# zhangganlin/GlORIE-SLAM

Measured on AMD Instinct MI355X. Metric: DSPO BA-update iters/sec + rendered rays/sec, 640x480 Replica keyframe graph, higher is better.
Workload: dtype f16 corr/ConvGRU, f32 Jacobians, f64 solve; render: f32 (decoder matmuls as 3-term f16 splits, f32 accumulate); 1 GPU; G8: 8 keyframes, 36 edges, 60x80 (640x480/8), BA itrs=2, DSPO stages alternating, context part of the GRU gates (one map per source keyframe) re-evaluated for all keyframes every 12 steps; multiview_filter.thresh = 0.25 (reference ships 0.01, configs/mono_point_slam.yaml:75: with untrained weights 0.01 rejects > 80 % of every frame and no depth_scale step would reach stage 2); render: 524k-point c; edges_local=36, edges_total=36, hw=4800, keyframes=8, parallelism=single GPU

## Files before the change

### glorie_slam_amd/csrc/conv.hip

```cpp
#include <hip/hip_runtime.h>
#include <stdint.h>
#include <stdlib.h>
#include <string.h>
#include <type_traits>
#include "common.hiph"

namespace glorie {

typedef __attribute__((ext_vector_type(8))) _Float16 f16x8;
typedef __attribute__((ext_vector_type(4))) _Float16 f16x4;
typedef __attribute__((ext_vector_type(4))) float f32x4;

enum { EPI_BIAS_ACT = 0, EPI_GRU_ZR = 1, EPI_GRU_Q = 2, EPI_GLO = 3, EPI_HEADS = 4, EPI_UPSAMPLE = 5 };
enum { CACT_NONE = 0, CACT_RELU = 1, CACT_SIGMOID = 2 };

struct ConvArgs {
  const _Float16* xa; int xa_stride; int cha;
  const _Float16* xb; int xb_stride; int chb;
  const _Float16* w;
  int taps, npad, nout;
  long P; int H, W, HW;
  _Float16* out; int out_stride;
  _Float16* out2; int out2_stride;
  const float* terms; int terms_stride; int act;
  const _Float16* net; int net_stride;
  const _Float16* z; int z_stride;
  const _Float16* pre; int pre_stride;
  const int* pre_map;
  long pbeg;
  int pair;
  unsigned long long* stamps;
  int pp_full, pp_nbr;
  const f16x8* tap_w; float* tap_out; int tap_groups, tap_ncols;
  const float* up_disps; const int64_t* up_ix; float* up_out; int up_f32;
};

constexpr int kTileN = 128;
constexpr long kConvPpwMinPixels = 512L * 512;

__device__ __forceinline__ float csigmoid(float x) { return __builtin_amdgcn_rcpf(1.0f + __expf(-x)); }
__device__ __forceinline__ float ctanh(float x) {
  const float e = __expf(-2.0f * fabsf(x));
  return copysignf((1.0f - e) * __builtin_amdgcn_rcpf(1.0f + e), x);
}

__device__ __forceinline__ void glds16(const void* src, char* lds_wave_base) {
  __builtin_amdgcn_global_load_lds((const __attribute__((address_space(1))) void*)src,
                                   (__attribute__((address_space(3))) void*)lds_wave_base, 16, 0, 0);
}

__device__ __forceinline__ long pre_pixel(const ConvArgs& a, long p) {
  if (!a.pre_map) return p;
  const int e = (int)(p / a.HW);
  return (long)a.pre_map[e] * a.HW + (p - (long)e * a.HW);
}

template <int EPI>
__device__ __forceinline__ void conv_epilogue(const ConvArgs& a, const f32x4 v, long p, int e, int n) {
  f16x4 o;
  if (EPI == EPI_BIAS_ACT) {
    float4 b = make_float4(0.f, 0.f, 0.f, 0.f);
    if (a.terms) b = *reinterpret_cast<const float4*>(a.terms + n);
    float f[4] = {v[0] + b.x, v[1] + b.y, v[2] + b.z, v[3] + b.w};
#pragma unroll
    for (int k = 0; k < 4; ++k) {
      if (a.act == CACT_RELU) f[k] = fmaxf(f[k], 0.0f);
      else if (a.act == CACT_SIGMOID) f[k] = csigmoid(f[k]);
      o[k] = (_Float16)f[k];
    }
    *reinterpret_cast<f16x4*>(a.out + p * a.out_stride + n) = o;
  } else if (EPI == EPI_GRU_ZR) {
    const float4 g = *reinterpret_cast<const float4*>(a.terms + (size_t)e * a.terms_stride + n);
    const float s[4] = {csigmoid(v[0] + g.x), csigmoid(v[1] + g.y), csigmoid(v[2] + g.z),
                        csigmoid(v[3] + g.w)};
    if (n < 128) {
#pragma unroll
      for (int k = 0; k < 4; ++k) o[k] = (_Float16)s[k];
      *reinterpret_cast<f16x4*>(a.out + p * a.out_stride + n) = o;
    } else {
      const f16x4 nv = *reinterpret_cast<const f16x4*>(a.net + p * a.net_stride + (n - 128));
#pragma unroll
      for (int k = 0; k < 4; ++k) o[k] = (_Float16)(s[k] * (float)nv[k]);
      *reinterpret_cast<f16x4*>(a.out2 + p * a.out2_stride + (n - 128)) = o;
    }
  } else {
    const float4 g = *reinterpret_cast<const float4*>(a.terms + (size_t)e * a.terms_stride + n);
    const f16x4 nv = *reinterpret_cast<const f16x4*>(a.net + p * a.net_stride + n);
    const f16x4 zv = *reinterpret_cast<const f16x4*>(a.z + p * a.z_stride + n);
    const float qv[4] = {ctanh(v[0] + g.x), ctanh(v[1] + g.y), ctanh(v[2] + g.z), ctanh(v[3] + g.w)};
#pragma unroll
    for (int k = 0; k < 4; ++k) {
      const float zz = (float)zv[k];
      o[k] = (_Float16)((1.0f - zz) * (float)nv[k] + zz * qv[k]);
    }
    *reinterpret_cast<f16x4*>(a.out + p * a.out_stride + n) = o;
  }
}

typedef __attribute__((ext_vector_type(2))) unsigned u32x2;

typedef __attribute__((ext_vector_type(4))) unsigned u32x4e;

template <int EPI, int MB, int NB>
__device__ __forceinline__ void conv_epilogue_pair(const ConvArgs& a, f32x4 (&acc)[MB][NB], long pbase, int nwave) {
  static_assert(MB % 2 == 0, "pairs of 16-row blocks");
  constexpr int PB = MB / 2;
  const int kg = (threadIdx.x & 63) >> 4;
  const __amdgpu_buffer_rsrc_t rO = __builtin_amdgcn_make_buffer_rsrc((void*)a.out, 0, 0x7fffffff, 0x00020000);
  const __amdgpu_buffer_rsrc_t rO2 = __builtin_amdgcn_make_buffer_rsrc((void*)(EPI == EPI_GRU_ZR ? a.out2 : a.out), 0,
                                                                      0x7fffffff, 0x00020000);
  const bool upper = EPI == EPI_GRU_ZR && nwave >= 128;
  const bool late = EPI != EPI_BIAS_ACT && a.pre;
  int nch[PB];
#pragma unroll
  for (int b = 0; b < PB; ++b) nch[b] = min(nwave + 32 * b + 8 * kg, a.nout - 8);
  float4 g[PB][2];
  int e_cur = -1;
  if (EPI == EPI_BIAS_ACT) {
#pragma unroll
    for (int b = 0; b < PB; ++b) {
      g[b][0] = a.terms ? *reinterpret_cast<const float4*>(a.terms + nch[b]) : make_float4(0.f, 0.f, 0.f, 0.f);
      g[b][1] = a.terms ? *reinterpret_cast<const float4*>(a.terms + nch[b] + 4) : make_float4(0.f, 0.f, 0.f, 0.f);
    }
// ... 183 lines not shown
    for (int rb = 0; rb < 2; ++rb) {
      f32x4 s = f32x4{0.f, 0.f, 0.f, 0.f};
#pragma unroll
      for (int c = 0; c < 2; ++c) s = __builtin_amdgcn_mfma_f32_16x16x32_f16(wf[c][rb], hf[c], s, 0, 0, 0);
      t[rb][ni] = s;
    }
  }
  float* red = reinterpret_cast<float*>(smem);
  __syncthreads();
  if (wm == 1) {
#pragma unroll
    for (int rb = 0; rb < 2; ++rb)
#pragma unroll
      for (int ni = 0; ni < NB; ++ni)
#pragma unroll
        for (int r = 0; r < 4; ++r) red[((wn * 8 + rb * 4 + ni) * 4 + r) * 64 + lane] = t[rb][ni][r];
  }
  __syncthreads();
  if (wm == 0) {
#pragma unroll
    for (int ni = 0; ni < NB; ++ni) {
      const long p = p0 + wn * 64 + ni * 16 + col;
      if (p >= a.P) continue;
      float* dst = a.tap_out + (size_t)(grp * a.tap_ncols) * a.P + p;
#pragma unroll
      for (int rb = 0; rb < 2; ++rb) {
        const int n = rb * 16 + kg * 4;
#pragma unroll
        for (int r = 0; r < 4; ++r) {
          const float v = t[rb][ni][r] + red[((wn * 8 + rb * 4 + ni) * 4 + r) * 64 + lane];
          if (n + r < a.tap_ncols) dst[(size_t)(n + r) * a.P] = v;
        }
      }
    }
  }
}

template <int MB, int NB>
__device__ __forceinline__ void conv_epilogue_glo(const ConvArgs& a, f32x4 (&acc)[MB][NB], long p0, long pbase, int wm,
                                                  int wn, int kg, int col, char* smem, int tile) {
  static_assert(MB == 4, "128-channel tile");
  const long pend = (p0 / a.HW + 1) * a.HW;
  float s0[MB][4];
#pragma unroll
  for (int mi = 0; mi < MB; ++mi)
#pragma unroll
    for (int k = 0; k < 4; ++k) s0[mi][k] = 0.0f;
  const int nb = wm * 64 + kg * 4;
#pragma unroll
  for (int ni = 0; ni < NB; ++ni) {
    const long p = pbase + ni * 16;
    const bool okp = p < pend;
    const long pc = okp ? p : pend - 1;
#pragma unroll
    for (int mi = 0; mi < MB; ++mi) {
      const int n = nb + mi * 16;
      const float4 b = *reinterpret_cast<const float4*>(a.terms + n);
      const f16x4 nv = *reinterpret_cast<const f16x4*>(a.net + pc * a.net_stride + n);
      const f32x4 v = acc[mi][ni];
      s0[mi][0] += okp ? csigmoid(v[0] + b.x) * (float)nv[0] : 0.0f;
      s0[mi][1] += okp ? csigmoid(v[1] + b.y) * (float)nv[1] : 0.0f;
      s0[mi][2] += okp ? csigmoid(v[2] + b.z) * (float)nv[2] : 0.0f;
      s0[mi][3] += okp ? csigmoid(v[3] + b.w) * (float)nv[3] : 0.0f;
    }
  }
#pragma unroll
  for (int mi = 0; mi < MB; ++mi)
#pragma unroll
    for (int k = 0; k < 4; ++k)
#pragma unroll
      for (int off = 8; off > 0; off >>= 1) s0[mi][k] += __shfl_xor(s0[mi][k], off, 64);
  float* red = reinterpret_cast<float*>(smem);
  __syncthreads();
  if (col == 0) {
#pragma unroll
    for (int mi = 0; mi < MB; ++mi)
#pragma unroll
      for (int k = 0; k < 4; ++k) red[wn * 128 + nb + mi * 16 + k] = s0[mi][k];
  }
  __syncthreads();
  const int tid = threadIdx.x;
  if (tid < 128) reinterpret_cast<float*>(a.out)[(size_t)tile * 128 + tid] = red[tid] + red[128 + tid];
}

__device__ __forceinline__ float round_prob(float v, bool f32) { return f32 ? v : (float)(_Float16)v; }

template <int MB, int NB>
__device__ __forceinline__ void conv_epilogue_upsample(const ConvArgs& a, f32x4 (&acc)[MB][NB], long p0, int n0, int wm,
                                                       int wn, int kg, int col, char* smem) {
  static_assert(MB == 4 && NB == 4, "128 x 128 tile");
  _Float16* T = reinterpret_cast<_Float16*>(smem);
  float4 bias[MB];
#pragma unroll
  for (int mi = 0; mi < MB; ++mi) bias[mi] = *reinterpret_cast<const float4*>(a.terms + n0 + wm * 64 + mi * 16 + kg * 4);
  __syncthreads();
#pragma unroll
  for (int ni = 0; ni < NB; ++ni) {
    const int pl = wn * 64 + ni * 16 + col;
#pragma unroll
    for (int mi = 0; mi < MB; ++mi) {
      const int b = wm * 4 + mi;
      const f32x4 v = acc[mi][ni];
      const f16x4 h = {(_Float16)(v[0] + bias[mi].x), (_Float16)(v[1] + bias[mi].y), (_Float16)(v[2] + bias[mi].z),
                       (_Float16)(v[3] + bias[mi].w)};
      *reinterpret_cast<f16x4*>(T + pl * 128 + ((b ^ (pl & 7)) * 16 + kg * 4)) = h;
    }
  }
  __syncthreads();
  const int tid = threadIdx.x;
  const int pl = tid & 127, hb = tid >> 7;
  const long p = p0 + pl;
  if (p >= a.P) return;
  const int asub = n0 >> 7;
  const int m = (int)(p / a.HW);
  const int q = (int)(p - (long)m * a.HW);
  const int y = q / a.W, x = q - y * a.W;
  const int frame = (int)a.up_ix[m];
  const float* dmap = a.up_disps + (size_t)frame * a.HW;
  float nb[9];
#pragma unroll
  for (int k = 0; k < 9; ++k) {
    const int yy = y + k / 3 - 1, xx = x + k % 3 - 1;
    const bool in = yy >= 0 && yy < a.H && xx >= 0 && xx < a.W;
    nb[k] = dmap[in ? yy * a.W + xx : q];
    if (!in) nb[k] = 0.0f;
  }
  float outv[4];
#pragma unroll
  for (int j = 0; j < 4; ++j) {
    const int b = hb * 4 + j;
    const f16x8* src = reinterpret_cast<const f16x8*>(T + pl * 128 + (b ^ (pl & 7)) * 16);
    const f16x8 lo = src[0], hi = src[1];
    float v[9];
#pragma unroll
    for (int k = 0; k < 8; ++k) v[k] = (float)lo[k];
    v[8] = (float)hi[0];
    float mx = v[0];
#pragma unroll
    for (int k = 1; k < 9; ++k) mx = fmaxf(mx, v[k]);
    float e[9], sum = 0.0f;
#pragma unroll
    for (int k = 0; k < 9; ++k) { e[k] = expf(v[k] - mx); sum += e[k]; }
    float o = 0.0f;
#pragma unroll
    for (int k = 0; k < 9; ++k)
      o = __fadd_rn(o, __fmul_rn(round_prob(e[k] / sum, a.up_f32 != 0), nb[k]));
    outv[j] = o;
  }
  float* dst = a.up_out + (size_t)frame * 64 * a.HW + (size_t)(8 * y + asub) * (8 * a.W) + 8 * x + hb * 4;
  *reinterpret_cast<float4*>(dst) = make_float4(outv[0], outv[1], outv[2], outv[3]);
}

template <int EPI, int NB, int BK, int NW, int ST, int MB = 4>
__global__ __launch_bounds__(64 * NW, (ST == 1 && MB * NB <= 16) ? 3 : 2) void conv_igemm_kernel(ConvArgs a) {
  constexpr int TN = 32 * MB;
  static_assert(ST == 1 || ST == 2, "LDS stages");
#if defined(__HIP_DEVICE_COMPILE__)
  constexpr int PT = (NW / 2) * 16 * NB;
  constexpr int RB = BK * 2;
  constexpr int SL = RB / 16;
  constexpr int RPI = 64 / SL;
  constexpr int XI = PT / RPI / NW;
  constexpr int WI = TN / RPI / NW;
  constexpr int XBYTES = PT * RB, WBYTES = TN * RB;
  constexpr int KK = BK / 32;
  extern __shared__ __attribute__((aligned(16))) char smem[];
  const int tid = threadIdx.x, lane = tid & 63, wv = tid >> 6;
  const int col = lane & 15, kg = lane >> 4;
// ... 911 lines not shown
  long rest_px = a.P - full_pt * 512;
  int nbr = 4;
  long rest_pt = 0;
  if (rest_px > 0) {
    const long per_cu = (rest_px * ntn + ncu - 1) / ncu;
    nbr = (int)((per_cu + 127) / 128);
    if (nbr > 4 || full_pt == 0) nbr = 4;
    if (nbr < 1) nbr = 1;
    rest_pt = (rest_px + 128 * nbr - 1) / (128 * nbr);
  }
  if (nbr == 4) { full_pt = pt_all; rest_pt = 0; }
  const long nwg = (full_pt + rest_pt) * ntn;
  if (nwg <= 0) return GLORIE_OK;
  if (nwg > 0x7fffffffL) return GLORIE_EINVAL;
  a.pp_full = (int)(full_pt * ntn);
  a.pp_nbr = nbr;
  const dim3 grid((unsigned)nwg);
  switch (epilogue) {
    case EPI_BIAS_ACT: launch_ppw_one<EPI_BIAS_ACT>(a, grid, st); break;
    case EPI_GRU_Q: launch_ppw_one<EPI_GRU_Q>(a, grid, st); break;
    case EPI_HEADS: launch_ppw_one<EPI_HEADS>(a, grid, st); break;
    default: return GLORIE_EUNSUPPORTED;
  }
  return check_launch();
}

template <int MB>
static int launch_conv_halo(const ConvArgs& a, int epilogue, hipStream_t st) {
  constexpr int PT = 128, TN = 32 * MB;
  if (a.pair && (MB % 2)) return GLORIE_EINVAL;
  const long ptiles = (a.P - a.pbeg + PT - 1) / PT;
  if (ptiles <= 0) return GLORIE_OK;
  const long nwg = ptiles * ((a.nout + TN - 1) / TN);
  if (nwg > 0x7fffffffL) return GLORIE_EINVAL;
  const dim3 grid((unsigned)nwg);
  const size_t lds = halo_lds_bytes(a.W, MB);
  switch (epilogue) {
    case EPI_BIAS_ACT: launch_halo_one<EPI_BIAS_ACT, MB>(a, grid, lds, st); break;
    case EPI_GRU_ZR: launch_halo_one<EPI_GRU_ZR, MB>(a, grid, lds, st); break;
    case EPI_GRU_Q:
      if constexpr (MB == 4) launch_halo_one<EPI_GRU_Q, MB>(a, grid, lds, st);
      else return GLORIE_EUNSUPPORTED;
      break;
    case EPI_HEADS:
      if constexpr (MB == 4) launch_halo_one<EPI_HEADS, MB>(a, grid, lds, st);
      else return GLORIE_EUNSUPPORTED;
      break;
    default: return GLORIE_EUNSUPPORTED;
  }
  return check_launch();
}

template <int NB, int BK, int NW, int ST, int MB = 4>
static int launch_conv(const ConvArgs& a, int epilogue, hipStream_t st, long max_ptiles = -1) {
  constexpr int PT = (NW / 2) * 16 * NB;
  if (a.pair && (MB % 2)) return GLORIE_EINVAL;
  long ptiles = (a.P - a.pbeg + PT - 1) / PT;
  if (epilogue == EPI_GLO) ptiles = (a.P / a.HW) * ((a.HW + PT - 1) / PT);
  if (max_ptiles >= 0) ptiles = ptiles < max_ptiles ? ptiles : max_ptiles;
  if (ptiles <= 0) return GLORIE_OK;
  const long nwg = ptiles * ((a.nout + 32 * MB - 1) / (32 * MB));
  if (nwg > 0x7fffffffL) return GLORIE_EINVAL;
  const dim3 grid((unsigned)nwg);
  switch (epilogue) {
    case EPI_BIAS_ACT: launch_one<EPI_BIAS_ACT, NB, BK, NW, ST, MB>(a, grid, st); break;
    case EPI_GRU_ZR: launch_one<EPI_GRU_ZR, NB, BK, NW, ST, MB>(a, grid, st); break;
    case EPI_GLO:
      if constexpr (MB == 4 && NB == 4 && NW == 4 && ST == 1) launch_one<EPI_GLO, NB, BK, NW, ST, MB>(a, grid, st);
      else return GLORIE_EUNSUPPORTED;
      break;
    case EPI_HEADS:
      if constexpr (MB == 4 && NB == 4 && NW == 4 && ST == 1) launch_one<EPI_HEADS, NB, BK, NW, ST, MB>(a, grid, st);
      else return GLORIE_EUNSUPPORTED;
      break;
    case EPI_UPSAMPLE:
      if constexpr (MB == 4 && NB == 4 && NW == 4 && ST == 1) launch_one<EPI_UPSAMPLE, NB, BK, NW, ST, MB>(a, grid, st);
      else return GLORIE_EUNSUPPORTED;
      break;
    default: launch_one<EPI_GRU_Q, NB, BK, NW, ST, MB>(a, grid, st); break;
  }
  return check_launch();
}

}

using namespace glorie;

static int conv_igemm_impl(const void* xa, int xa_stride, int ca, const void* xb, int xb_stride,
                           int cb, const void* w_packed, int taps, int nout, int epilogue,
                           const float* terms, int terms_stride, int act, const void* net,
                           int net_stride, const void* z, int z_stride, void* out, int out_stride,
                           void* out2, int out2_stride, const void* pre, int pre_stride, const int* pre_map,
                           int N, int H, int W, void* stream, const void* tap_w, float* tap_out, int tap_groups,
                           int tap_ncols, const float* up_disps = nullptr, const int64_t* up_ix = nullptr,
                           float* up_out = nullptr, int up_f32 = 0) {
  if (N < 0 || H <= 0 || W <= 0 || (taps != 1 && taps != 9) || nout <= 0 || (nout & 3)) return GLORIE_EINVAL;
  if (ca < 0 || cb < 0 || (ca % 64) || (cb % 64) || ca + cb == 0) return GLORIE_EINVAL;
  const int pair = (epilogue >> 8) & 1;
  const int policy = (epilogue >> 12) & 15;
  epilogue &= 0xff;
  if (policy > 7) return GLORIE_EINVAL;
  if (epilogue < 0 || epilogue > 5) return GLORIE_EINVAL;
  if (pair && (epilogue > EPI_GRU_Q || (nout & 31))) return GLORIE_EINVAL;
  if (epilogue == EPI_UPSAMPLE && (!up_disps || !up_ix || !up_out || !terms || nout != 1024 || taps != 1 || pre))
    return GLORIE_EINVAL;
  if (epilogue == EPI_HEADS && (!tap_w || !tap_out || !terms || tap_groups < 1 || tap_ncols < 1 || tap_ncols > 32 ||
                                nout < 128 * tap_groups || (nout & 127) || act != CACT_RELU || pre))
    return GLORIE_EINVAL;
  if (N == 0) return GLORIE_OK;
  if ((ca && (!xa || (xa_stride & 7))) || (cb && (!xb || (xb_stride & 7)))) return GLORIE_EINVAL;
  if (!w_packed || !out || (out_stride & 3)) return GLORIE_EINVAL;
  if (epilogue == EPI_GRU_ZR && (nout != 256 || !terms || !net || !out2 || (terms_stride & 3))) return GLORIE_EINVAL;
  if (epilogue == EPI_GRU_Q && (nout != 128 || !terms || !net || !z || (terms_stride & 3))) return GLORIE_EINVAL;
  if (pre && (epilogue == EPI_BIAS_ACT || epilogue == EPI_GLO || (pre_stride & 3))) return GLORIE_EINVAL;
  if (epilogue == EPI_GLO && (nout != 128 || taps != 1 || !terms || !net)) return GLORIE_EINVAL;
  ConvArgs a;
  a.xa = reinterpret_cast<const _Float16*>(xa); a.xa_stride = xa_stride; a.cha = ca / 64;
  a.xb = reinterpret_cast<const _Float16*>(xb); a.xb_stride = xb_stride; a.chb = cb / 64;
  a.w = reinterpret_cast<const _Float16*>(w_packed);
  a.taps = taps; a.nout = nout; a.npad = (nout + kTileN - 1) / kTileN * kTileN;
  a.P = (long)N * H * W; a.H = H; a.W = W; a.HW = H * W;
  a.out = reinterpret_cast<_Float16*>(out); a.out_stride = out_stride;
  a.out2 = reinterpret_cast<_Float16*>(out2); a.out2_stride = out2_stride;
  a.terms = terms; a.terms_stride = terms_stride; a.act = act;
  a.net = reinterpret_cast<const _Float16*>(net); a.net_stride = net_stride;
  a.z = reinterpret_cast<const _Float16*>(z); a.z_stride = z_stride;
  a.pre = reinterpret_cast<const _Float16*>(pre); a.pre_stride = pre_stride; a.pre_map = pre ? pre_map : nullptr;
  a.pbeg = 0;
  a.tap_w = reinterpret_cast<const f16x8*>(tap_w); a.tap_out = tap_out; a.tap_groups = tap_groups;
  a.tap_ncols = tap_ncols;
  a.up_disps = up_disps; a.up_ix = up_ix; a.up_out = up_out; a.up_f32 = up_f32;
  a.pair = pair;
  a.pp_full = 0; a.pp_nbr = 4;
#ifdef EXP_CONV_STAMPS
  a.stamps = getenv("GLORIE_CONV_STAMPS") ? (unsigned long long*)strtoull(getenv("GLORIE_CONV_STAMPS"), nullptr, 0) : nullptr;
#else
  a.stamps = nullptr;
#endif
  const long lim = 0x7fffffffL;
  if (((a.P + W + 2) * (long)xa_stride + 64) * 2 > lim || ((a.P + W + 2) * (long)xb_stride + 64) * 2 > lim ||
      ((long)taps * a.npad * (ca + cb) + 64) * 2 > lim || (pre && (a.P * (long)pre_stride + 512) * 2 > lim) ||
      (a.P * (long)out_stride + nout) * 2 > lim || (out2 && (a.P * (long)out2_stride + 128) * 2 > lim))
    return GLORIE_EINVAL;
  hipStream_t st = (hipStream_t)stream;
  if (policy == 6) return launch_conv_pp(a, epilogue, st);
  if (policy == 7) return launch_conv_ppw(a, epilogue, st);
  {
    const char* ppw = getenv("GLORIE_CONV_PPW");
    const bool fits = (nout & 127) == 0 && (epilogue == EPI_BIAS_ACT || epilogue == EPI_GRU_Q || epilogue == EPI_HEADS);
    const bool want = ppw ? ppw[0] == '1' : (taps == 9 && (nout == 128 || epilogue == EPI_HEADS) && epilogue != EPI_BIAS_ACT &&
                                             a.P >= kConvPpwMinPixels);
    if (policy == 0 && fits && want && !(ppw && ppw[0] == '0')) return launch_conv_ppw(a, epilogue, st);
  }
  {
    if (policy == 0 && taps == 9 && a.pbeg == 0) {
      const long tiles128 = (a.P + 127) / 128 * ((nout + 127) / 128);
      if (nout > 64 && (nout & 255) != 0 && W <= 83 && (epilogue <= EPI_GRU_Q || epilogue == EPI_HEADS) &&
          !(epilogue == EPI_BIAS_ACT && tiles128 <= 384))
        return launch_conv_halo<4>(a, epilogue, st);
    }
  }
  if (epilogue == EPI_HEADS || epilogue == EPI_UPSAMPLE) return launch_conv<4, 64, 4, 1>(a, epilogue, st);
  if (nout <= 64 && epilogue == EPI_BIAS_ACT) return launch_conv<4, 64, 4, 1, 2>(a, epilogue, st);
  const int ntn = (nout + 127) / 128;
  const long slots128 = 3L * 256;
  const long full_rounds = ((a.P + 127) / 128 * ntn) / slots128;
  const long pt_a = full_rounds * slots128 / ntn;
  const char t0c = policy == 1 ? '1' : policy == 2 ? '6' : policy == 3 ? 's' : policy == 4 ? 'w' : 0;
  if (policy == 0 && (nout & 255) == 0 && taps == 9 && epilogue <= EPI_GRU_ZR && a.P >= 256L * 256)
    return launch_conv_pp(a, epilogue, st);
  if (t0c == 0 && (nout & 255) == 0) return launch_conv<4, 64, 4, 1, 8>(a, epilogue, st);
  if (t0c == 0 && epilogue == EPI_BIAS_ACT && (a.P + 127) / 128 * ntn <= 384) return launch_conv<2, 64, 4, 1>(a, epilogue, st);
  if (t0c == 0 && epilogue == EPI_BIAS_ACT && taps == 1) return launch_conv<2, 64, 4, 1>(a, epilogue, st);
  if (t0c == 'w') return launch_conv<8, 64, 4, 1, 4>(a, epilogue, st);
  if (t0c == '6') return launch_conv<2, 64, 4, 1>(a, epilogue, st);
  if (t0c == 's' && full_rounds >= 1) {
    const int rc_a = launch_conv<4, 64, 4, 1>(a, epilogue, st, pt_a);
    if (rc_a != GLORIE_OK) return rc_a;
    a.pbeg = pt_a * 128;
    return a.pbeg < a.P ? launch_conv<2, 64, 4, 1>(a, epilogue, st) : GLORIE_OK;
  }
  return launch_conv<4, 64, 4, 1>(a, epilogue, st);
}

extern "C" int glorie_conv_igemm(const void* xa, int xa_stride, int ca, const void* xb, int xb_stride,
                                 int cb, const void* w_packed, int taps, int nout, int epilogue,
                                 const float* terms, int terms_stride, int act, const void* net,
                                 int net_stride, const void* z, int z_stride, void* out, int out_stride,
                                 void* out2, int out2_stride, const void* pre, int pre_stride, const int* pre_map,
                                 int N, int H, int W, void* stream) {
  if ((epilogue & 0xff) == EPI_HEADS || (epilogue & 0xff) == EPI_UPSAMPLE) return GLORIE_EINVAL;
  return conv_igemm_impl(xa, xa_stride, ca, xb, xb_stride, cb, w_packed, taps, nout, epilogue, terms, terms_stride, act,
                         net, net_stride, z, z_stride, out, out_stride, out2, out2_stride, pre, pre_stride, pre_map, N, H,
                         W, stream, nullptr, nullptr, 0, 0);
}

extern "C" int glorie_conv_igemm_heads(const void* x, int x_stride, int c, const void* w_packed, int taps, int nout,
                                       const float* bias, const void* tap_w, int groups, int K, float* tap_out,
                                       void* out, int out_stride, int N, int H, int W, void* stream) {
  if (K < 1 || K > 3 || groups < 1 || groups > 4) return GLORIE_EINVAL;
  if (nout > 128 * groups && !out) return GLORIE_EINVAL;
  void* o = out ? out : (void*)tap_out;
  return conv_igemm_impl(x, x_stride, c, nullptr, 0, 0, w_packed, taps, nout, EPI_HEADS, bias, 0, CACT_RELU, nullptr, 0,
                         nullptr, 0, o, out ? out_stride : 4, nullptr, 0, nullptr, 0, nullptr, N, H, W, stream, tap_w,
                         tap_out, groups, 9 * K);
}

extern "C" int glorie_conv_upsample(const void* x, int x_stride, int c, const void* w_packed, const float* bias,
                                    const float* disps, const int64_t* ix, float* disps_up, int softmax_f32, int M,
                                    int H, int W, void* stream) {
  if (!disps || !ix || !disps_up || !bias) return GLORIE_EINVAL;
  return conv_igemm_impl(x, x_stride, c, nullptr, 0, 0, w_packed, 1, 1024, EPI_UPSAMPLE, bias, 0, CACT_NONE, nullptr, 0,
                         nullptr, 0, disps_up, 4, nullptr, 0, nullptr, 0, nullptr, M, H, W, stream, nullptr, nullptr, 0,
                         0, disps, ix, disps_up, softmax_f32);
}
```

### glorie_slam_amd/csrc/gru.hip

```cpp
#include <hip/hip_runtime.h>
#include <stdint.h>
#include "common.hiph"

namespace glorie {

typedef __attribute__((ext_vector_type(8))) _Float16 h8;

__device__ __forceinline__ float sigmoidf_(float x) { return 1.0f / (1.0f + __expf(-x)); }
__device__ __forceinline__ float tanhf_(float x) {
  const float e = __expf(-2.0f * fabsf(x));
  const float t = (1.0f - e) / (1.0f + e);
  return copysignf(t, x);
}

enum { ACT_NONE = 0, ACT_RELU = 1, ACT_SIGMOID = 2, ACT_SOFTPLUS = 3 };

template <int C8T>
__global__ __launch_bounds__(256) void bias_act_kernel(const _Float16* __restrict__ x, int xs,
                                                       const float* __restrict__ bias,
                                                       _Float16* __restrict__ y, int ys, long P,
                                                       int C8R, int act) {
  const int C8 = C8T ? C8T : C8R;
  const long idx = (long)blockIdx.x * 256 + threadIdx.x;
  if (idx >= P * C8) return;
// ... 190 lines not shown
                                                        const float* __restrict__ in_bias, int in_relu,
                                                        const f16x8* __restrict__ wp,
                                                        float* __restrict__ taps, int ncols, int tstride,
                                                        long P) {
  const int lane = threadIdx.x & 63, wv = threadIdx.x >> 6;
  const int col = lane & 15, kg = lane >> 4;
  const int grp = blockIdx.y;
  f16x8 bfrag[NT][4];
#pragma unroll
  for (int t = 0; t < NT; ++t)
#pragma unroll
    for (int kk = 0; kk < 4; ++kk) bfrag[t][kk] = wp[(((size_t)grp * NT + t) * 4 + kk) * 64 + lane];
  float ib[4][8];
#pragma unroll
  for (int kk = 0; kk < 4; ++kk)
#pragma unroll
    for (int k = 0; k < 8; ++k) ib[kk][k] = in_bias ? in_bias[grp * 128 + kk * 32 + kg * 8 + k] : 0.0f;
  const long ntiles = (P + 15) / 16;
  for (long tile = (long)blockIdx.x * 4 + wv; tile < ntiles; tile += (long)gridDim.x * 4) {
    const long p0 = tile * 16;
    const long pa = min(p0 + col, P - 1);
    const f16x8* src = reinterpret_cast<const f16x8*>(x + pa * xs + grp * 128 + kg * 8);
    f16x8 afrag[4];
#pragma unroll
    for (int kk = 0; kk < 4; ++kk) afrag[kk] = src[kk * 4];
    if (in_bias || in_relu) {
#pragma unroll
      for (int kk = 0; kk < 4; ++kk)
#pragma unroll
        for (int k = 0; k < 8; ++k) {
          float f = (float)afrag[kk][k] + ib[kk][k];
          if (in_relu) f = fmaxf(f, 0.0f);
          afrag[kk][k] = (_Float16)f;
        }
    }
#pragma unroll
    for (int t = 0; t < NT; ++t) {
      f32x4 acc = f32x4{0.f, 0.f, 0.f, 0.f};
#pragma unroll
      for (int kk = 0; kk < 4; ++kk)
        acc = __builtin_amdgcn_mfma_f32_16x16x32_f16(afrag[kk], bfrag[t][kk], acc, 0, 0, 0);
      const int n = t * 16 + col;
      if (n < ncols) {
#pragma unroll
        for (int r = 0; r < 4; ++r) {
          const long pr = p0 + kg * 4 + r;
          if (pr < P) taps[pr * tstride + grp * ncols + n] = acc[r];
        }
      }
    }
  }
}

__device__ __forceinline__ float softplusf_(float x) { return x > 20.0f ? x : log1pf(__expf(x)); }

template <bool PLANAR>
__global__ __launch_bounds__(256) void conv_stencil_kernel(const float* __restrict__ taps, int ncols,
                                                           int tstride, const float* __restrict__ bias,
                                                           int K, int groups, int act_packed, float scale,
                                                           float* __restrict__ out, long P, int H, int W,
                                                           float* __restrict__ out_last = nullptr) {
  const long idx = (long)blockIdx.x * 256 + threadIdx.x;
  if (idx >= P * K * groups) return;
  const int gk = PLANAR ? (int)(idx / P) : (int)(idx % (K * groups));
  const long p = PLANAR ? idx - (long)gk * P : idx / (K * groups);
  const int grp = gk / K, j = gk - grp * K;
  const int xw = (int)(p % W), yh = (int)((p / W) % H);
  float acc = bias ? bias[grp * K + j] : 0.0f;
#pragma unroll
  for (int d = 0; d < 9; ++d) {
    const int dy = d / 3 - 1, dx = d % 3 - 1;
    if ((unsigned)(yh + dy) < (unsigned)H && (unsigned)(xw + dx) < (unsigned)W)
      acc += PLANAR ? taps[(size_t)(grp * ncols + d * K + j) * P + (p + dy * W + dx)]
                    : taps[(p + dy * W + dx) * tstride + grp * ncols + d * K + j];
  }
  const int act = (act_packed >> (4 * grp)) & 15;
  if (act == ACT_RELU) acc = fmaxf(acc, 0.0f);
  else if (act == ACT_SIGMOID) acc = sigmoidf_(acc);
  else if (act == ACT_SOFTPLUS) acc = softplusf_(acc);
  if (out_last && grp == groups - 1) out_last[(size_t)p * K + j] = acc * scale;
  else out[((size_t)grp * P + p) * K + j] = acc * scale;
}

}

using namespace glorie;

extern "C" int glorie_bias_act(const void* x, int x_stride, const float* bias, void* y, int y_stride,
                               long P, int C, int act, void* stream) {
  if (P < 0 || C <= 0 || (C & 7) || (x_stride & 7) || (y_stride & 7)) return GLORIE_EINVAL;
  if (P == 0) return GLORIE_OK;
  if (!x || !y) return GLORIE_EINVAL;
  const long total = P * (C / 8);
  const dim3 grid((unsigned)((total + 255) / 256));
  auto launch = [&](auto kernel) {
    hipLaunchKernelGGL(kernel, grid, dim3(256), 0, (hipStream_t)stream,
                       reinterpret_cast<const _Float16*>(x), x_stride, bias,
                       reinterpret_cast<_Float16*>(y), y_stride, P, C / 8, act);
  };
  switch (C / 8) {
    case 8: launch(bias_act_kernel<8>); break;
    case 16: launch(bias_act_kernel<16>); break;
    case 48: launch(bias_act_kernel<48>); break;
    default: launch(bias_act_kernel<0>); break;
  }
  return check_launch();
}

__global__ __launch_bounds__(128) void glo_from_tiles_kernel(const float* __restrict__ tiles, const float* __restrict__ G,
                                                             const float* __restrict__ Gb, int M,
                                                             float* __restrict__ g, int HW) {
  __shared__ float glo[128];
  const int n = blockIdx.x;
  const int tpm = (HW + 127) >> 7;
  const float* tp = tiles + (size_t)n * tpm * 128 + threadIdx.x;
  float s = 0.0f;
  int t = 0;
  for (; t + 8 <= tpm; t += 8) {
    float v[8];
#pragma unroll
    for (int k = 0; k < 8; ++k) v[k] = tp[(size_t)(t + k) * 128];
#pragma unroll
    for (int k = 0; k < 8; ++k) s += v[k];
  }
  for (; t < tpm; ++t) s += tp[(size_t)t * 128];
  const int o = blockIdx.y * 128 + threadIdx.x;
  const int oc = min(o, M - 1);
  float gv[16];
#pragma unroll
  for (int k = 0; k < 16; ++k) gv[k] = G[(size_t)k * M + oc];
  glo[threadIdx.x] = s / (float)HW;
  __syncthreads();
  if (o >= M) return;
  float acc0 = Gb[o], acc1 = 0.0f, acc2 = 0.0f, acc3 = 0.0f;
#pragma unroll
  for (int c0 = 0; c0 < 128; c0 += 16) {
    float nx[16];
    if (c0 + 16 < 128) {
#pragma unroll
      for (int k = 0; k < 16; ++k) nx[k] = G[(size_t)(c0 + 16 + k) * M + o];
    }
#pragma unroll
    for (int k = 0; k < 16; k += 4) {
      acc0 = fmaf(glo[c0 + k], gv[k], acc0);
      acc1 = fmaf(glo[c0 + k + 1], gv[k + 1], acc1);
      acc2 = fmaf(glo[c0 + k + 2], gv[k + 2], acc2);
      acc3 = fmaf(glo[c0 + k + 3], gv[k + 3], acc3);
    }
    if (c0 + 16 < 128) {
#pragma unroll
      for (int k = 0; k < 16; ++k) gv[k] = nx[k];
    }
  }
  g[(size_t)n * M + o] = (acc0 + acc1) + (acc2 + acc3);
}

extern "C" int glorie_gru_glo_from_tiles(const float* tiles, const float* G, const float* Gb, int M, float* g, int N,
                                         int HW, void* stream) {
  if (N < 0 || HW < 1 || M <= 0) return GLORIE_EINVAL;
  if (N == 0) return GLORIE_OK;
  if (!tiles || !G || !Gb || !g) return GLORIE_EINVAL;
  hipLaunchKernelGGL(glo_from_tiles_kernel, dim3(N, (M + 127) / 128), dim3(128), 0, (hipStream_t)stream, tiles, G, Gb, M,
                     g, HW);
  return check_launch();
}

// ... 12 lines not shown
}

extern "C" int glorie_gru_gate_zr(const void* zr, int zr_stride, const float* g, int g_stride,
                                  const void* net, int n_stride, void* z, int z_stride, void* rnet, int r_stride,
                                  int N, int HW, void* stream) {
  if (N < 0 || HW <= 0) return GLORIE_EINVAL;
  if (N == 0) return GLORIE_OK;
  if (!zr || !g || !net || !z || !rnet) return GLORIE_EINVAL;
  const long P = (long)N * HW;
  hipLaunchKernelGGL(gru_gate_zr_kernel, dim3((unsigned)((P * 16 + 255) / 256)), dim3(256), 0,
                     (hipStream_t)stream, reinterpret_cast<const _Float16*>(zr), zr_stride, g, g_stride,
                     reinterpret_cast<const _Float16*>(net), n_stride, reinterpret_cast<_Float16*>(z),
                     z_stride, reinterpret_cast<_Float16*>(rnet), r_stride, P, HW);
  return check_launch();
}

extern "C" int glorie_gru_gate_q(const void* qc, int q_stride, const float* gq, int gq_stride,
                                 const void* z, int z_stride, const void* net, int n_stride, void* out,
                                 int o_stride, void* out2, int o2_stride, int N, int HW, void* stream) {
  if (N < 0 || HW <= 0) return GLORIE_EINVAL;
  if (N == 0) return GLORIE_OK;
  if (!qc || !gq || !z || !net || !out) return GLORIE_EINVAL;
  const long P = (long)N * HW;
  hipLaunchKernelGGL(gru_gate_q_kernel, dim3((unsigned)((P * 16 + 255) / 256)), dim3(256), 0,
                     (hipStream_t)stream, reinterpret_cast<const _Float16*>(qc), q_stride, gq, gq_stride,
                     reinterpret_cast<const _Float16*>(z), z_stride, reinterpret_cast<const _Float16*>(net),
                     n_stride, reinterpret_cast<_Float16*>(out), o_stride,
                     reinterpret_cast<_Float16*>(out2), o2_stride, P, HW);
  return check_launch();
}

__global__ __launch_bounds__(256) void update_bookkeeping_kernel(
    const float* __restrict__ coords1, const float* __restrict__ delta, float* __restrict__ target, long n_target,
    const float* __restrict__ eta, const int64_t* __restrict__ frames, float* __restrict__ damping_table,
    float* __restrict__ damping_ba, long n_eta, int HW, float ep, int64_t* __restrict__ age, int n_edges) {
#pragma clang fp contract(off)
  const long i = (long)blockIdx.x * 256 + threadIdx.x;
  if (i < n_target) target[i] = coords1[i] + delta[i];
  if (i < n_eta) {
    const float e = eta[i];
    const long g = i / HW;
    damping_table[(size_t)frames[g] * HW + (i - g * HW)] = e;
    const float m = e * 0.2f;
    damping_ba[i] = m + ep;
  }
  if (age && i < n_edges) age[i] += 1;
}

extern "C" int glorie_update_bookkeeping(const float* coords1, const float* delta, float* target, long n_target,
                                         const float* eta, const int64_t* frames, float* damping_table,
                                         float* damping_ba, int G, int HW, float ep, int64_t* age, int n_edges,
                                         void* stream) {
  if (n_target < 0 || G < 0 || HW <= 0 || n_edges < 0) return GLORIE_EINVAL;
  const long n_eta = (long)G * HW;
  const long n_age = age ? (long)n_edges : 0;
  long n = n_target > n_eta ? n_target : n_eta;
  if (n_age > n) n = n_age;
  if (n == 0) return GLORIE_OK;
  if ((n_target && (!coords1 || !delta || !target)) || (n_eta && (!eta || !frames || !damping_table || !damping_ba)))
    return GLORIE_EINVAL;
  hipLaunchKernelGGL(update_bookkeeping_kernel, dim3((unsigned)((n + 255) / 256)), dim3(256), 0, (hipStream_t)stream,
                     coords1, delta, target, n_target, eta, frames, damping_table, damping_ba, n_eta, HW, ep, age, n_edges);
  return check_launch();
}

extern "C" int glorie_segment_mean(const void* x, int x_stride, const float* bias, int relu,
                                   const int64_t* ix, int N, void* out, int o_stride, int G, int HW,
                                   void* stream) {
  if (N < 0 || G < 0 || HW <= 0 || (x_stride & 7) || (o_stride & 7)) return GLORIE_EINVAL;
  if (G == 0) return GLORIE_OK;
  if (!out || (N > 0 && (!x || !ix))) return GLORIE_EINVAL;
  hipLaunchKernelGGL(segment_mean_kernel, dim3((HW * 16 + 255) / 256, G), dim3(256), 0,
                     (hipStream_t)stream, reinterpret_cast<const _Float16*>(x), x_stride, bias, relu,
                     ix, N, reinterpret_cast<_Float16*>(out), o_stride, HW);
  return check_launch();
}

extern "C" int glorie_conv3x3_small(const void* x, int x_stride, const float* in_bias, int in_relu,
                                    const void* w_packed, const float* out_bias, int groups, int K,
                                    int act_packed, float scale, float* taps, float* out, int N, int H,
                                    int W, void* stream) {
  if (N < 0 || H <= 0 || W <= 0 || groups < 1 || groups > 4 || K < 1 || K > 3 || (x_stride & 7))
    return GLORIE_EINVAL;
  if (N == 0) return GLORIE_OK;
  if (!x || !w_packed || !taps || !out) return GLORIE_EINVAL;
  const long P = (long)N * H * W;
  const int ncols = 9 * K, tstride = ncols * groups;
  const long ntiles = (P + 15) / 16;
  const unsigned gx = (unsigned)min((ntiles + 3) / 4, (long)2048);
  hipStream_t st = (hipStream_t)stream;
  if (ncols <= 16)
    hipLaunchKernelGGL(conv_taps_kernel<1>, dim3(gx, groups), dim3(256), 0, st,
                       reinterpret_cast<const _Float16*>(x), x_stride, in_bias, in_relu,
                       reinterpret_cast<const f16x8*>(w_packed), taps, ncols, tstride, P);
  else
    hipLaunchKernelGGL(conv_taps_kernel<2>, dim3(gx, groups), dim3(256), 0, st,
                       reinterpret_cast<const _Float16*>(x), x_stride, in_bias, in_relu,
                       reinterpret_cast<const f16x8*>(w_packed), taps, ncols, tstride, P);
  const long total = P * K * groups;
  hipLaunchKernelGGL(conv_stencil_kernel<false>, dim3((unsigned)((total + 255) / 256)), dim3(256), 0, st, taps,
                     ncols, tstride, out_bias, K, groups, act_packed, scale, out, P, H, W);
  return check_launch();
}

extern "C" int glorie_conv_stencil(const float* taps, const float* out_bias, int groups, int K, int act_packed,
                                   float scale, float* out, float* out_last, int N, int H, int W, void* stream) {
  if (N < 0 || H <= 0 || W <= 0 || groups < 1 || groups > 4 || K < 1 || K > 3) return GLORIE_EINVAL;
  if (N == 0) return GLORIE_OK;
  if (!taps || !out) return GLORIE_EINVAL;
  const long P = (long)N * H * W, total = P * K * groups;
  hipLaunchKernelGGL(conv_stencil_kernel<true>, dim3((unsigned)((total + 255) / 256)), dim3(256), 0, (hipStream_t)stream,
                     taps, 9 * K, 9 * K * groups, out_bias, K, groups, act_packed, scale, out, P, H, W, out_last);
  return check_launch();
}
```

Baseline: 929.2 BA-update iters/s.

## Add dedicated 1x1 conv kernels for GLO/upsample and fused single-output 3x3 conv

Adds a new conv1x1 source file with a persistent-grid GLO kernel, which fuses sigmoid gating and tile reduction with software-prefetched buffer loads, and an upsample kernel that fuses the logits MFMA with the convex-upsampling softmax. It also adds a fused single-output 3x3 conv kernel (groups=1, K=1) that computes taps into LDS and applies the stencil in one launch, replacing the two-kernel taps+stencil path. The 3x3 path is on by default. The 1x1 GLO/upsample paths are used only with GLORIE_CONV1X1=1 or policy 8. The aim is fewer launches and fewer global round-trips for small-channel convs, at the cost of halo recomputation and LDS pressure.

```diff
diff --git a/glorie_slam_amd/csrc/conv.hip b/glorie_slam_amd/csrc/conv.hip
--- a/glorie_slam_amd/csrc/conv.hip
+++ b/glorie_slam_amd/csrc/conv.hip
@@ -4,6 +4,7 @@
 #include <string.h>
 #include <type_traits>
 #include "common.hiph"
+#include "conv1x1.hiph"
 
 namespace glorie {
 
@@ -38,7 +39,6 @@
 constexpr int kTileN = 128;
 constexpr long kConvPpwMinPixels = 512L * 512;
 
-__device__ __forceinline__ float csigmoid(float x) { return __builtin_amdgcn_rcpf(1.0f + __expf(-x)); }
 __device__ __forceinline__ float ctanh(float x) {
   const float e = __expf(-2.0f * fabsf(x));
   return copysignf((1.0f - e) * __builtin_amdgcn_rcpf(1.0f + e), x);
@@ -388,8 +388,6 @@
   const int tid = threadIdx.x;
   if (tid < 128) reinterpret_cast<float*>(a.out)[(size_t)tile * 128 + tid] = red[tid] + red[128 + tid];
 }
-
-__device__ __forceinline__ float round_prob(float v, bool f32) { return f32 ? v : (float)(_Float16)v; }
 
 template <int MB, int NB>
 __device__ __forceinline__ void conv_epilogue_upsample(const ConvArgs& a, f32x4 (&acc)[MB][NB], long p0, int n0, int wm,
@@ -1467,6 +1465,11 @@
   return check_launch();
 }
 
+static char env_switch(const char* name) {
+  const char* v = getenv(name);
+  return v ? v[0] : 0;
+}
+
 }
 
 using namespace glorie;
@@ -1484,7 +1487,7 @@
   const int pair = (epilogue >> 8) & 1;
   const int policy = (epilogue >> 12) & 15;
   epilogue &= 0xff;
-  if (policy > 7) return GLORIE_EINVAL;
+  if (policy > 8) return GLORIE_EINVAL;
   if (epilogue < 0 || epilogue > 5) return GLORIE_EINVAL;
   if (pair && (epilogue > EPI_GRU_Q || (nout & 31))) return GLORIE_EINVAL;
   if (epilogue == EPI_UPSAMPLE && (!up_disps || !up_ix || !up_out || !terms || nout != 1024 || taps != 1 || pre))
@@ -1518,7 +1521,8 @@
   a.pair = pair;
   a.pp_full = 0; a.pp_nbr = 4;
 #ifdef EXP_CONV_STAMPS
-  a.stamps = getenv("GLORIE_CONV_STAMPS") ? (unsigned long long*)strtoull(getenv("GLORIE_CONV_STAMPS"), nullptr, 0) : nullptr;
+  static const char* const stamps_env = getenv("GLORIE_CONV_STAMPS");
+  a.stamps = stamps_env ? (unsigned long long*)strtoull(stamps_env, nullptr, 0) : nullptr;
 #else
   a.stamps = nullptr;
 #endif
@@ -1528,14 +1532,31 @@
       (a.P * (long)out_stride + nout) * 2 > lim || (out2 && (a.P * (long)out2_stride + 128) * 2 > lim))
     return GLORIE_EINVAL;
   hipStream_t st = (hipStream_t)stream;
+  if (policy == 8 || (policy == 0 && (epilogue == EPI_GLO || epilogue == EPI_UPSAMPLE))) {
+    static const char sw = env_switch("GLORIE_CONV1X1");
+    const bool fits = (epilogue == EPI_GLO || epilogue == EPI_UPSAMPLE) && taps == 1 && ca == 128 && cb == 0;
+    if (policy == 8 && !fits) return GLORIE_EUNSUPPORTED;
+    if (fits && (policy == 8 || sw == '1')) {
+      Conv1x1Args s;
+      s.x = a.xa; s.x_stride = xa_stride; s.w = a.w; s.bias = terms;
+      s.P = a.P; s.H = H; s.W = W; s.HW = a.HW;
+      s.net = a.net; s.net_stride = net_stride; s.tiles = reinterpret_cast<float*>(out);
+      s.up_disps = up_disps; s.up_ix = up_ix; s.up_out = up_out; s.up_f32 = up_f32;
+      const int rc = epilogue == EPI_GLO ? launch_conv1x1_glo(s, st) : launch_conv1x1_upsample(s, st);
+      if (rc != GLORIE_EUNSUPPORTED || policy == 8) return rc;
+    }
+  }
   if (policy == 6) return launch_conv_pp(a, epilogue, st);
   if (policy == 7) return launch_conv_ppw(a, epilogue, st);
   {
-    const char* ppw = getenv("GLORIE_CONV_PPW");
+    const char ppw = env_switch("GLORIE_CONV_PPW");
     const bool fits = (nout & 127) == 0 && (epilogue == EPI_BIAS_ACT || epilogue == EPI_GRU_Q || epilogue == EPI_HEADS);
-    const bool want = ppw ? ppw[0] == '1' : (taps == 9 && (nout == 128 || epilogue == EPI_HEADS) && epilogue != EPI_BIAS_ACT &&
-                                             a.P >= kConvPpwMinPixels);
-    if (policy == 0 && fits && want && !(ppw && ppw[0] == '0')) return launch_conv_ppw(a, epilogue, st);
+    const bool want = ppw ? ppw == '1' : (taps == 9 && (nout == 128 || epilogue == EPI_HEADS) && epilogue != EPI_BIAS_ACT &&
+                                          a.P >= kConvPpwMinPixels);
+    if (policy == 0 && fits && want) {
+      const int rc = launch_conv_ppw(a, epilogue, st);
+      if (rc != GLORIE_EUNSUPPORTED || !ppw) return rc;
+    }
   }
   {
     if (policy == 0 && taps == 9 && a.pbeg == 0) {
@@ -1595,7 +1616,9 @@
                                     const float* disps, const int64_t* ix, float* disps_up, int softmax_f32, int M,
                                     int H, int W, void* stream) {
   if (!disps || !ix || !disps_up || !bias) return GLORIE_EINVAL;
-  return conv_igemm_impl(x, x_stride, c, nullptr, 0, 0, w_packed, 1, 1024, EPI_UPSAMPLE, bias, 0, CACT_NONE, nullptr, 0,
-                         nullptr, 0, disps_up, 4, nullptr, 0, nullptr, 0, nullptr, M, H, W, stream, nullptr, nullptr, 0,
-                         0, disps, ix, disps_up, softmax_f32);
-}
+  const int policy = (softmax_f32 >> 12) & 15;
+  if (policy != 0 && policy != 1 && policy != 8) return GLORIE_EINVAL;
+  return conv_igemm_impl(x, x_stride, c, nullptr, 0, 0, w_packed, 1, 1024, EPI_UPSAMPLE | (policy << 12), bias, 0, CACT_NONE,
+                         nullptr, 0, nullptr, 0, disps_up, 4, nullptr, 0, nullptr, 0, nullptr, M, H, W, stream, nullptr,
+                         nullptr, 0, 0, disps, ix, disps_up, (softmax_f32 & 0xfff) != 0);
+}
diff --git a/glorie_slam_amd/csrc/conv1x1.hip b/glorie_slam_amd/csrc/conv1x1.hip
--- /dev/null
+++ b/glorie_slam_amd/csrc/conv1x1.hip
@@ -0,0 +1,247 @@
+#include <hip/hip_runtime.h>
+#include <stdint.h>
+#include "common.hiph"
+#include "conv1x1.hiph"
+
+namespace glorie {
+
+typedef __attribute__((ext_vector_type(8))) _Float16 f16x8;
+typedef __attribute__((ext_vector_type(4))) _Float16 f16x4;
+typedef __attribute__((ext_vector_type(4))) float f32x4;
+typedef __attribute__((ext_vector_type(4))) unsigned u32x4s;
+typedef __attribute__((ext_vector_type(2))) unsigned u32x2s;
+
+__global__ __launch_bounds__(256, 3) void conv1x1_glo_kernel(Conv1x1Args a, int ntiles, int tpm) {
+#if defined(__HIP_DEVICE_COMPILE__)
+  constexpr int MB = 2;
+  const int tid = threadIdx.x, lane = tid & 63, wv = tid >> 6;
+  const int col = lane & 15, kg = lane >> 4;
+  const int ch0 = wv * 32;
+  f16x8 wf[MB][4];
+#pragma unroll
+  for (int mi = 0; mi < MB; ++mi)
+#pragma unroll
+    for (int ks = 0; ks < 4; ++ks)
+      wf[mi][ks] = *reinterpret_cast<const f16x8*>(a.w + (size_t)(ch0 + mi * 16 + col) * 128 + ks * 32 + kg * 8);
+  float4 b[MB];
+#pragma unroll
+  for (int mi = 0; mi < MB; ++mi) b[mi] = *reinterpret_cast<const float4*>(a.bias + ch0 + mi * 16 + kg * 4);
+
+  const __amdgpu_buffer_rsrc_t rX = __builtin_amdgcn_make_buffer_rsrc((void*)a.x, 0, 0x7fffffff, 0x00020000);
+  const __amdgpu_buffer_rsrc_t rN = __builtin_amdgcn_make_buffer_rsrc((void*)a.net, 0, 0x7fffffff, 0x00020000);
+  const int stride = gridDim.x;
+  int tile = blockIdx.x;
+  if (tile >= ntiles) return;
+
+  auto tile_range = [&](int t, int& p0, int& pend) {
+    t = min(t, ntiles - 1);
+    const int m = t / tpm;
+    p0 = m * a.HW + (t - m * tpm) * 128;
+    pend = (m + 1) * a.HW;
+  };
+  u32x4s xr[4][4];
+  u32x2s nr[4][MB];
+  bool okr[4];
+  auto issue = [&](int set, int p0, int pend, int blk) {
+    const int p = p0 + blk * 16 + col;
+    okr[set] = p < pend;
+    const int pc = okr[set] ? p : pend - 1;
+    const unsigned xo = (unsigned)((pc * a.x_stride + kg * 8) * 2);
+    const unsigned no = (unsigned)((pc * a.net_stride + ch0 + kg * 4) * 2);
+#pragma unroll
+    for (int ks = 0; ks < 4; ++ks) xr[set][ks] = __builtin_amdgcn_raw_buffer_load_b128(rX, xo, ks * 64, 0);
+#pragma unroll
+    for (int mi = 0; mi < MB; ++mi) nr[set][mi] = __builtin_amdgcn_raw_buffer_load_b64(rN, no, mi * 32, 0);
+  };
+
+  int p0c, pendc, p0n, pendn;
+  tile_range(tile, p0c, pendc);
+  tile_range(tile + stride, p0n, pendn);
+  constexpr int kAhead = 2;
+#pragma unroll
+  for (int blk = 0; blk < kAhead; ++blk) issue(blk, p0c, pendc, blk);
+  while (true) {
+    float s0[MB][4], h0[MB][4];
+#pragma unroll
+    for (int blk = 0; blk < 8; ++blk) {
+      if (blk + kAhead < 8) issue((blk + kAhead) & 3, p0c, pendc, blk + kAhead);
+      else issue((blk + kAhead) & 3, p0n, pendn, blk + kAhead - 8);
+      __builtin_amdgcn_sched_barrier(0);
+      const int set = blk & 3;
+      if ((blk & 3) == 0) {
+#pragma unroll
+        for (int mi = 0; mi < MB; ++mi)
+#pragma unroll
+          for (int k = 0; k < 4; ++k) s0[mi][k] = 0.0f;
+      }
+      f32x4 acc[MB];
+#pragma unroll
+      for (int mi = 0; mi < MB; ++mi) acc[mi] = f32x4{0.f, 0.f, 0.f, 0.f};
+#pragma unroll
+      for (int ks = 0; ks < 4; ++ks) {
+        const f16x8 xf = __builtin_bit_cast(f16x8, xr[set][ks]);
+#pragma unroll
+        for (int mi = 0; mi < MB; ++mi) acc[mi] = __builtin_amdgcn_mfma_f32_16x16x32_f16(wf[mi][ks], xf, acc[mi], 0, 0, 0);
+      }
+      const bool okp = okr[set];
+#pragma unroll
+      for (int mi = 0; mi < MB; ++mi) {
+        const f16x4 nv = __builtin_bit_cast(f16x4, nr[set][mi]);
+        const f32x4 v = acc[mi];
+        s0[mi][0] += okp ? csigmoid(v[0] + b[mi].x) * (float)nv[0] : 0.0f;
+        s0[mi][1] += okp ? csigmoid(v[1] + b[mi].y) * (float)nv[1] : 0.0f;
+        s0[mi][2] += okp ? csigmoid(v[2] + b[mi].z) * (float)nv[2] : 0.0f;
+        s0[mi][3] += okp ? csigmoid(v[3] + b[mi].w) * (float)nv[3] : 0.0f;
+      }
+      if ((blk & 3) == 3) {
+#pragma unroll
+        for (int mi = 0; mi < MB; ++mi)
+#pragma unroll
+          for (int k = 0; k < 4; ++k) {
+#pragma unroll
+            for (int off = 8; off > 0; off >>= 1) s0[mi][k] += __shfl_xor(s0[mi][k], off, 64);
+            if (blk == 3) h0[mi][k] = s0[mi][k];
+          }
+      }
+    }
+    if (col == 0) {
+      float* dst = a.tiles + (size_t)tile * 128 + ch0 + kg * 4;
+#pragma unroll
+      for (int mi = 0; mi < MB; ++mi)
+        *reinterpret_cast<float4*>(dst + mi * 16) =
+            make_float4(h0[mi][0] + s0[mi][0], h0[mi][1] + s0[mi][1], h0[mi][2] + s0[mi][2], h0[mi][3] + s0[mi][3]);
+    }
+    tile += stride;
+    if (tile >= ntiles) return;
+    p0c = p0n; pendc = pendn;
+    tile_range(tile + stride, p0n, pendn);
+  }
+#endif
+}
+
+__global__ __launch_bounds__(512, 1) void conv1x1_upsample_kernel(Conv1x1Args a, int nblk) {
+#if defined(__HIP_DEVICE_COMPILE__)
+  __shared__ __attribute__((aligned(16))) _Float16 smem[8][16 * 128];
+  const int tid = threadIdx.x, lane = tid & 63, wv = tid >> 6;
+  const int col = lane & 15, kg = lane >> 4;
+  f16x8 wf[8][4];
+#pragma unroll
+  for (int mi = 0; mi < 8; ++mi)
+#pragma unroll
+    for (int ks = 0; ks < 4; ++ks)
+      wf[mi][ks] = *reinterpret_cast<const f16x8*>(a.w + (size_t)(wv * 128 + mi * 16 + col) * 128 + ks * 32 + kg * 8);
+  const float* bias = a.bias + wv * 128 + kg * 4;
+  _Float16* T = smem[wv];
+
+  const __amdgpu_buffer_rsrc_t rX = __builtin_amdgcn_make_buffer_rsrc((void*)a.x, 0, 0x7fffffff, 0x00020000);
+  const int P = (int)a.P;
+  constexpr unsigned kDropped = 0x80000000u;
+  auto issue = [&](u32x4s (&r)[4], int blk) {
+    const int p = blk * 16 + col;
+    const unsigned xo = (blk < nblk && p < P) ? (unsigned)((p * a.x_stride + kg * 8) * 2) : kDropped;
+#pragma unroll
+    for (int ks = 0; ks < 4; ++ks) r[ks] = __builtin_amdgcn_raw_buffer_load_b128(rX, xo, ks * 64, 0);
+  };
+  auto logits = [&](const u32x4s (&r)[4]) {
+    f16x8 xf[4];
+#pragma unroll
+    for (int ks = 0; ks < 4; ++ks) xf[ks] = __builtin_bit_cast(f16x8, r[ks]);
+#pragma unroll
+    for (int mi = 0; mi < 8; ++mi) {
+      f32x4 v = f32x4{0.f, 0.f, 0.f, 0.f};
+#pragma unroll
+      for (int ks = 0; ks < 4; ++ks) v = __builtin_amdgcn_mfma_f32_16x16x32_f16(wf[mi][ks], xf[ks], v, 0, 0, 0);
+      const float4 bb = *reinterpret_cast<const float4*>(bias + mi * 16);
+      const f16x4 h = {(_Float16)(v[0] + bb.x), (_Float16)(v[1] + bb.y), (_Float16)(v[2] + bb.z), (_Float16)(v[3] + bb.w)};
+      *reinterpret_cast<f16x4*>(T + col * 128 + ((mi ^ (col & 7)) * 16 + kg * 4)) = h;
+    }
+    __builtin_amdgcn_fence(__ATOMIC_RELEASE, "wavefront");
+    __builtin_amdgcn_wave_barrier();
+    __builtin_amdgcn_fence(__ATOMIC_ACQUIRE, "wavefront");
+  };
+  auto upsample = [&](int blk) {
+    const int pl = lane >> 2, hb = lane & 3;
+    const int p = blk * 16 + pl;
+    if (p < P) {
+      const int m = p / a.HW;
+      const int q = p - m * a.HW;
+      const int y = q / a.W, x = q - y * a.W;
+      const int frame = (int)a.up_ix[m];
+      const float* dmap = a.up_disps + (size_t)frame * a.HW;
+      float nb[9];
+#pragma unroll
+      for (int k = 0; k < 9; ++k) {
+        const int yy = y + k / 3 - 1, xx = x + k % 3 - 1;
+        const bool in = yy >= 0 && yy < a.H && xx >= 0 && xx < a.W;
+        nb[k] = dmap[in ? yy * a.W + xx : q];
+        if (!in) nb[k] = 0.0f;
+      }
+      float outv[2];
+#pragma unroll
+      for (int j = 0; j < 2; ++j) {
+        const int bsub = hb * 2 + j;
+        const _Float16* src = T + pl * 128 + (bsub ^ (pl & 7)) * 16;
+        const f16x8 lo = *reinterpret_cast<const f16x8*>(src);
+        float v[9];
+#pragma unroll
+        for (int k = 0; k < 8; ++k) v[k] = (float)lo[k];
+        v[8] = (float)src[8];
+        float mx = v[0];
+#pragma unroll
+        for (int k = 1; k < 9; ++k) mx = fmaxf(mx, v[k]);
+        float e[9], sum = 0.0f;
+#pragma unroll
+        for (int k = 0; k < 9; ++k) { e[k] = expf(v[k] - mx); sum += e[k]; }
+        float o = 0.0f;
+#pragma unroll
+        for (int k = 0; k < 9; ++k)
+          o = __fadd_rn(o, __fmul_rn(round_prob(e[k] / sum, a.up_f32 != 0), nb[k]));
+        outv[j] = o;
+      }
+      float* dst = a.up_out + (size_t)frame * 64 * a.HW + (size_t)(8 * y + wv) * (8 * a.W) + 8 * x + hb * 2;
+      *reinterpret_cast<float2*>(dst) = make_float2(outv[0], outv[1]);
+    }
+    __builtin_amdgcn_fence(__ATOMIC_RELEASE, "wavefront");
+    __builtin_amdgcn_wave_barrier();
+    __builtin_amdgcn_fence(__ATOMIC_ACQUIRE, "wavefront");
+  };
+
+  u32x4s r[4];
+  int blk = blockIdx.x;
+  if (blk >= nblk) return;
+  const int step = gridDim.x;
+  issue(r, blk);
+  while (true) {
+    logits(r);
+    issue(r, blk + step);
+    upsample(blk);
+    blk += step;
+    if (blk >= nblk) return;
+  }
+#endif
+}
+
+static bool fits_31_bits(long rows, int stride_halfs) { return (rows * (long)stride_halfs + 128) * 2 < 0x7fffffffL; }
+
+int launch_conv1x1_glo(const Conv1x1Args& a, hipStream_t st) {
+  if (a.P <= 0) return GLORIE_OK;
+  if ((a.x_stride & 7) || (a.net_stride & 3) || a.P >= 0x7fffffffL || !fits_31_bits(a.P, a.x_stride) ||
+      !fits_31_bits(a.P, a.net_stride))
+    return GLORIE_EUNSUPPORTED;
+  const long tpm = (a.HW + 127) / 128, ntiles = (a.P / a.HW) * tpm;
+  if (ntiles >= 0x7fffffffL / 128) return GLORIE_EUNSUPPORTED;
+  const long cap = 3L * device_cus();
+  hipLaunchKernelGGL(conv1x1_glo_kernel, dim3((unsigned)(ntiles < cap ? ntiles : cap)), dim3(256), 0, st, a, (int)ntiles,
+                     (int)tpm);
+  return check_launch();
+}
+
+int launch_conv1x1_upsample(const Conv1x1Args& a, hipStream_t st) {
+  if (a.P <= 0) return GLORIE_OK;
+  if ((a.x_stride & 7) || a.P >= 0x7fffffffL || !fits_31_bits(a.P, a.x_stride)) return GLORIE_EUNSUPPORTED;
+  const long nblk = (a.P + 15) / 16, cap = device_cus();
+  hipLaunchKernelGGL(conv1x1_upsample_kernel, dim3((unsigned)(nblk < cap ? nblk : cap)), dim3(512), 0, st, a, (int)nblk);
+  return check_launch();
+}
+
+}
diff --git a/glorie_slam_amd/csrc/gru.hip b/glorie_slam_amd/csrc/gru.hip
--- a/glorie_slam_amd/csrc/gru.hip
+++ b/glorie_slam_amd/csrc/gru.hip
@@ -296,6 +296,71 @@
   else out[((size_t)grp * P + p) * K + j] = acc * scale;
 }
 
+constexpr int kSmallTile = 128;
+__global__ __launch_bounds__(256) void conv3x3_one_kernel(const _Float16* __restrict__ x, int xs,
+                                                          const float* __restrict__ in_bias, int in_relu,
+                                                          const f16x8* __restrict__ wp, const float* __restrict__ bias,
+                                                          int act, float scale, float* __restrict__ out, long P, int H,
+                                                          int W) {
+  extern __shared__ float tap_rows[];
+  const int lane = threadIdx.x & 63, wv = threadIdx.x >> 6;
+  const int col = lane & 15, kg = lane >> 4;
+  f16x8 bfrag[4];
+#pragma unroll
+  for (int kk = 0; kk < 4; ++kk) bfrag[kk] = wp[kk * 64 + lane];
+  float ib[4][8];
+#pragma unroll
+  for (int kk = 0; kk < 4; ++kk)
+#pragma unroll
+    for (int k = 0; k < 8; ++k) ib[kk][k] = in_bias ? in_bias[kk * 32 + kg * 8 + k] : 0.0f;
+  const long t0 = (long)blockIdx.x * kSmallTile;
+  const long h0 = max(t0 - (W + 1), 0L), h1 = min(t0 + kSmallTile + W + 1, P);
+  const int nblk = (int)((h1 - h0 + 15) / 16);
+  for (int blk = wv; blk < nblk; blk += 4) {
+    const long p0 = h0 + blk * 16;
+    const long pa = min(p0 + col, P - 1);
+    const f16x8* src = reinterpret_cast<const f16x8*>(x + pa * xs + kg * 8);
+    f16x8 afrag[4];
+#pragma unroll
+    for (int kk = 0; kk < 4; ++kk) afrag[kk] = src[kk * 4];
+    if (in_bias || in_relu) {
+#pragma unroll
+      for (int kk = 0; kk < 4; ++kk)
+#pragma unroll
+        for (int k = 0; k < 8; ++k) {
+          float f = (float)afrag[kk][k] + ib[kk][k];
+          if (in_relu) f = fmaxf(f, 0.0f);
+          afrag[kk][k] = (_Float16)f;
+        }
+    }
+    f32x4 acc = f32x4{0.f, 0.f, 0.f, 0.f};
+#pragma unroll
+    for (int kk = 0; kk < 4; ++kk) acc = __builtin_amdgcn_mfma_f32_16x16x32_f16(afrag[kk], bfrag[kk], acc, 0, 0, 0);
+    if (col < 9) {
+#pragma unroll
+      for (int r = 0; r < 4; ++r) {
+        const long pr = p0 + kg * 4 + r;
+        if (pr < h1) tap_rows[(pr - h0) * 9 + col] = acc[r];
+      }
+    }
+  }
+  __syncthreads();
+  const long p = t0 + threadIdx.x;
+  if (threadIdx.x >= kSmallTile || p >= P) return;
+  const int xw = (int)(p % W), yh = (int)((p / W) % H);
+  float acc = bias ? bias[0] : 0.0f;
+#pragma unroll
+  for (int d = 0; d < 9; ++d) {
+    const int dy = d / 3 - 1, dx = d % 3 - 1;
+    if ((unsigned)(yh + dy) < (unsigned)H && (unsigned)(xw + dx) < (unsigned)W)
+      acc += tap_rows[(p + dy * W + dx - h0) * 9 + d];
+  }
+  if (act == ACT_RELU) acc = fmaxf(acc, 0.0f);
+  else if (act == ACT_SIGMOID) acc = sigmoidf_(acc);
+  else if (act == ACT_SOFTPLUS) acc = softplusf_(acc);
+  out[p] = acc * scale;
+}
+
 }
 
 using namespace glorie;
@@ -474,6 +539,9 @@
                                     int W, void* stream) {
   if (N < 0 || H <= 0 || W <= 0 || groups < 1 || groups > 4 || K < 1 || K > 3 || (x_stride & 7))
     return GLORIE_EINVAL;
+  const int policy = (in_relu >> 12) & 15;
+  in_relu = (in_relu & 0xfff) != 0;
+  if (policy != 0 && policy != 1 && policy != 8) return GLORIE_EINVAL;
   if (N == 0) return GLORIE_OK;
   if (!x || !w_packed || !taps || !out) return GLORIE_EINVAL;
   const long P = (long)N * H * W;
@@ -481,6 +549,19 @@
   const long ntiles = (P + 15) / 16;
   const unsigned gx = (unsigned)min((ntiles + 3) / 4, (long)2048);
   hipStream_t st = (hipStream_t)stream;
+  {
+    static const char* const sw = getenv("GLORIE_CONV1X1");
+    const size_t lds = (size_t)(kSmallTile + 2 * (W + 1)) * 9 * sizeof(float);
+    const long wgs = (P + kSmallTile - 1) / kSmallTile;
+    const bool fits = groups == 1 && K == 1 && lds <= 64 * 1024 && wgs <= 0x7fffffffL;
+    if (policy == 8 && !fits) return GLORIE_EUNSUPPORTED;
+    if (fits && (policy == 8 || (policy == 0 && !(sw && sw[0] == '0')))) {
+      hipLaunchKernelGGL(conv3x3_one_kernel, dim3((unsigned)wgs), dim3(256), lds, st, reinterpret_cast<const _Float16*>(x),
+                         x_stride, in_bias, in_relu, reinterpret_cast<const f16x8*>(w_packed), out_bias, act_packed & 15,
+                         scale, out, P, H, W);
+      return check_launch();
+    }
+  }
   if (ncols <= 16)
     hipLaunchKernelGGL(conv_taps_kernel<1>, dim3(gx, groups), dim3(256), 0, st,
                        reinterpret_cast<const _Float16*>(x), x_stride, in_bias, in_relu,
```

Measured after the change: 930.8 BA-update iters/s, median of 4. About the same (+0.2%).
